# Gepeng18/Sentinel

Measured on AMD Instinct MI355X. Metric: admission decisions/sec at 1M rules Zipf(1.1), 1/2/4/8 GPU; % HBM peak, higher is better.
Workload: dtype int64

## Files before the change

### sentinel_amd/csrc/cluster.hip

```cpp
#include "cluster.hpp"
#include "cluster_exact.hpp"
#include "cparam_exact.hpp"

#include <cstdio>
#include <cstdlib>

#include <algorithm>
#include <type_traits>

namespace sga {

namespace {

constexpr int kThreads = 256;
constexpr int kItems = 16;
constexpr int kTileElems = kThreads * kItems;

enum : uint8_t { RUN_FAST = 0, RUN_DONE = 1 };

__device__ __forceinline__ uint64_t lanemask_lt64(int lane) { return (1ULL << lane) - 1ULL; }

__device__ __forceinline__ HashEntry slot_lookup(const ClusterState &st, int64_t fid) {
    uint32_t h = (uint32_t)hash_flow_id(fid) & st.hmask;
    for (uint32_t probe = 0; probe <= st.hmask; ++probe) {
// ... 1489 lines not shown
    const uint32_t hi = (uint32_t)__builtin_amdgcn_readlane((int)(uint32_t)((uint64_t)v >> 32), l);
    return (int64_t)(((uint64_t)hi << 32) | lo);
}

__device__ __forceinline__ uint32_t rank_hot(uint32_t *cw, uint32_t hid) {
    const uint32_t sh = (hid & 1u) << 4;
    return (atomicAdd(&cw[hid >> 1], 1u << sh) >> sh) & 0xFFFFu;
}


__device__ __forceinline__ uint32_t hot_count(const BatchScratch &sc) {
    return min(sc.hot_ctl[0], (uint32_t)kHot);
}

__device__ __forceinline__ uint32_t bucket_delta(uint32_t t, uint32_t W, uint32_t r0, double inv) {
    const uint64_t x = (uint64_t)r0 + t;
    int64_t q = (int64_t)((double)x * inv);
    const int64_t r = (int64_t)x - q * (int64_t)W;
    if (r < 0) --q;
    else if (r >= (int64_t)W) ++q;
    return (uint32_t)q;
}

__global__ __launch_bounds__(kThreads) void k_hot_precheck(ClusterState st, BatchScratch sc, const ReqIn in,
                                                           int64_t ts_base, uint32_t n, int pipelined) {
    if (blockIdx.x == 0 && st.dense_n) {
        const uint32_t W = st.wtab[threadIdx.x];
        WConst wc;
        wc.W = W;
        wc.r0 = (uint32_t)(ts_base % (int64_t)W);
        wc.inv = 1.0 / (double)W;
        sc.wconst[threadIdx.x] = wc;
    }
    const uint32_t h = blockIdx.x * kThreads + threadIdx.x;
    if (h < (uint32_t)kHot) {
        sc.plo[h] = 0;
        sc.phi[h] = 0;
    }
    if (h >= hot_count(sc) || n == 0) return;
    const int64_t W = (int64_t)sc.hot_ctl[2];
    const int64_t t0 = ts_base + (int64_t)in.ts_at(0);
    if (pipelined && h == 0 && t0 < (int64_t)*sc.tmax_all) atomicOr(&sc.counters[CTL_FLAGS], kFlagState);
    const int64_t ws0 = t0 - t0 % W;
    const uint32_t s = sc.hot_slot[h];
    const SlotParam P = st.param[s];
    bool bad = P.W != (int32_t)W || !P.active || P.S <= 1 || P.S > 64;
    const Rec R = rec_of(st, P);
    for (int j = 0; j < P.S && !bad; ++j) {
        const int64_t w = R.start(j);
        if (w != kAbsent && w > ws0) bad = true;
    }
    if (bad) atomicOr(&sc.counters[CTL_FLAGS], kFlagState);
}

constexpr uint32_t kKeyHot = 1u << 19;
constexpr uint32_t kPsGroups = 256;
constexpr int kKeyWaves = kHotSeg / kSubSeg;
constexpr int kKeyThreads = kKeyWaves * 64;
static_assert(kKeyWaves == kSubPerSeg, "one wave per compaction segment");
struct KeyShared {
    WConst wcs[256];
    uint16_t cnt[kKeyWaves][kHot];
    uint32_t s_np[kKeyWaves], s_bd[kKeyWaves], s_tm[kKeyWaves];
    uint32_t s_bmin, s_bmax;
    union {
        uint32_t hist0[2][256];
        uint32_t phist[kPartBins];
    };
};
template <int kPass, bool kDense, bool kNT = false, bool kPk = false>
__device__ __forceinline__ void hot_key(KeyShared &sh, const ClusterState &st, const BatchScratch &sc, const ReqIn in,
                                        int64_t ts_base, uint32_t n, uint64_t *__restrict__ out, int dbg,
                                        int d0, uint32_t *__restrict__ hist, uint32_t ntiles) {
    const int64_t *__restrict__ flow_id = in.flow;
    const int32_t *__restrict__ acquire = in.acq;
    const uint8_t *__restrict__ prio = in.prio;
    const uint32_t *__restrict__ ts_off = in.ts;
    const uint32_t *__restrict__ pk = in.pk;
    WConst *wcs = sh.wcs;
    const int pl = d0 < 0 ? -d0 : 0;
    if (pl) d0 = 0;
    const uint32_t dmask = (1u << d0) - 1u;
    auto &cnt = sh.cnt;
    uint32_t *s_np = sh.s_np, *s_bd = sh.s_bd;
    const uint32_t flags0 = sc.counters[CTL_FLAGS];
    if (kPass == 0 && (flags0 & kFlagState)) return;
    if (kPass == 1 && !(flags0 & (kFlagRerun | kFlagState))) return;
    const uint32_t nhot = kPass == 0 ? hot_count(sc) : 0u;
    const int lane = threadIdx.x & 63, wave = threadIdx.x >> 6;
    const uint64_t lt = lanemask_lt64(lane);
    if (kDense)
        for (int k = threadIdx.x; k < 256; k += kKeyThreads) wcs[k] = sc.wconst[k];
    for (int k = threadIdx.x; k < (pl ? kPartBins : 2 * 256); k += kKeyThreads) sh.phist[k] = 0;
    if (nhot) {
        uint4 *cz = reinterpret_cast<uint4 *>(&cnt[0][0]);
        for (int k = threadIdx.x; k < (int)(sizeof(cnt) / 16); k += kKeyThreads) cz[k] = make_uint4(0, 0, 0, 0);
    }
    if (threadIdx.x == 0) {
        sh.s_bmin = 0xFFFFFFFFu;
        sh.s_bmax = 0u;
    }
    __syncthreads();
    const uint32_t seg = blockIdx.x;
    const uint32_t sub = seg * kKeyWaves + wave;
    const uint32_t ubase = sub * kSubSeg;
    const bool active = ubase < n;
    uint16_t *c = cnt[wave];
    const uint32_t Wh = nhot ? sc.hot_ctl[2] : 1u;
    const uint32_t r0h = (uint32_t)(ts_base % (int64_t)Wh);
    const double invh = 1.0 / (double)Wh;
    const uint32_t Wc = (kDense && sc.hot_ctl[0]) ? sc.hot_ctl[2] : 1u;
    const uint32_t r0c = (uint32_t)(ts_base % (int64_t)Wc);
    const double invc = 1.0 / (double)Wc;
    uint32_t wflags = 0, nc = 0, np = 0, bdmax = 0, tmax_l = 0;
    const uint32_t send = min(n, ubase + (uint32_t)kSubSeg);
    uint32_t hc[kSubRounds];
#pragma unroll
    for (int r = 0; r < kSubRounds; ++r) hc[r] = kNoCode;
    if (active) {
        uint32_t ptso = ubase > 0 ? (kPk ? pk[3 * (size_t)(ubase - 1) + 1] : ts_off[ubase - 1]) : 0u;
        uint32_t pbd = (nhot && ubase > 0) ? min(bucket_delta(ptso, Wh, r0h, invh), (uint32_t)kHotBuckets - 1) : 0u;
        const bool use_prio = kPk || prio != nullptr;
        constexpr int nchunks = kSubRounds / kH1Chunk;
        struct Buf {
            int64_t f[kH1Chunk];
            int32_t a[kH1Chunk];
            uint32_t t[kH1Chunk], p[kH1Chunk], d[kH1Chunk], m[kH1Chunk];
            HashEntry e[kH1Chunk];
        };
        Buf B0, B1, B2;
        const uint8_t *pr_src = kPk ? nullptr : (use_prio ? prio : reinterpret_cast<const uint8_t *>(acquire));
        auto load = [&](int ch, Buf &B) {
#pragma unroll
            for (int u = 0; u < kH1Chunk; ++u) {
                const uint32_t i = min(ubase + (uint32_t)(ch * kH1Chunk + u) * 64 + lane, n - 1);
                if (kPk) {
                    const uint32_t *r = pk + 3 * (size_t)i;
                    uint32_t w0, w1, w2;
                    if (kNT) {
                        w0 = __builtin_nontemporal_load(r);
                        w1 = __builtin_nontemporal_load(r + 1);
                        w2 = __builtin_nontemporal_load(r + 2);
                    } else {
                        w0 = r[0];
                        w1 = r[1];
                        w2 = r[2];
// ... 127 lines not shown
                    ptso = lane_u32(B.t[u], 63);
                    if (valid && q >= (uint32_t)kHotBuckets) wflags |= kFlagBucket;
                    const uint32_t bdh = min(q, (uint32_t)kHotBuckets - 1);
                    if (valid) bdmax = max(bdmax, bdh);
                    if (i == 0) sc.counters[CTL_BDLO] = bdh;
                    const uint32_t pbk = wave_shr1(bdh, pbd);
                    if (valid && hp && bdh > pbk) {
                        for (uint32_t qq = pbk + 1; qq <= bdh; ++qq) sc.hbnd[qq] = i;
                        if (i & (uint32_t)(kHotSeg - 1)) {
                            atomicMin(&sh.s_bmin, pbk + 1);
                            atomicMax(&sh.s_bmax, bdh);
                        }
                    }
                    pbd = lane_u32(bdh, 63);
                    if (valid) hc[ch * kH1Chunk + u] = (kind == 2 ? (kKeyHot | hid | (p << 12)) : 0u) | (bdh << 13);
                }
                const bool emit = kind == 1;
                const uint64_t em = __ballot(emit);
                if (emit) {
                    if (kNT)
                        __builtin_nontemporal_store(el_pack(slot, bd6, p, a7, i),
                                                    &sc.el_tile[(size_t)ubase + nc + (uint32_t)__popcll(em & lt)]);
                    else
                        sc.el_tile[(size_t)ubase + nc + (uint32_t)__popcll(em & lt)] = el_pack(slot, bd6, p, a7, i);
                    if (d0) atomicAdd(&sh.hist0[wave >> 2][slot & dmask], 1u);
                    if (pl) atomicAdd(&sh.phist[slot >> pl], 1u);
                }
                nc += (uint32_t)__popcll(em);
            }
        };
        load(0, B0);
        lookup(B0);
        load(1, B1);
#pragma unroll
        for (int ch = 0; ch < nchunks; ch += 3) {
            lookup(B1);
            load(ch + 2, B2);
            process(B0, ch);
            if (ch + 1 >= nchunks) break;
            lookup(B2);
            load(ch + 3, B0);
            process(B1, ch + 1);
            if (ch + 2 >= nchunks) break;
            lookup(B0);
            load(ch + 4, B1);
            process(B2, ch + 2);
        }
        if (nhot && !(dbg & 4)) {
#pragma unroll
            for (int r = 0; r < kSubRounds; ++r) {
                const uint32_t i = ubase + (uint32_t)r * 64 + lane;
                const uint32_t kv = hc[r];
                const bool hot = i < send && (kv & kKeyHot);
                const uint32_t hid = kv & 0xFFFu, p = (kv >> 12) & 1u, bdh = (kv >> 13) & 63u;
                uint32_t r_in = 0;
                if (hot) r_in = rank_hot(reinterpret_cast<uint32_t *>(c), hid);
                np += (uint32_t)__popcll(__ballot(hot && p));
                hc[r] = hot ? ((p << 31) | hid | (r_in << 12) | (bdh << 25)) : kNoCode;
            }
        }
    }
    if (wflags) atomicOr(&sc.counters[CTL_FLAGS], wflags);
    if (nhot) {
bdmax = wave_max_u32(bdmax);
        if (lane == 0) {
            s_np[wave] = np;
            s_bd[wave] = bdmax;
        }
        __syncthreads();
        {
            uint32_t *cw = reinterpret_cast<uint32_t *>(&cnt[0][0]);
            uint32_t *row = reinterpret_cast<uint32_t *>(sc.hcnt + (size_t)seg * kHot);
            for (uint32_t k = threadIdx.x; k < (nhot + 1) / 2; k += kKeyThreads) {
                uint32_t run = 0;
#pragma unroll
                for (int w = 0; w < kKeyWaves; ++w) {
                    const uint32_t v = cw[w * (kHot / 2) + k];
                    cw[w * (kHot / 2) + k] = run;
                    run += v;
                }
                row[k] = run;
            }
        }
        if (threadIdx.x == 0) {
            uint32_t a = 0, m = 0;
            for (int w = 0; w < kKeyWaves; ++w) {
                a += s_np[w];
                m = max(m, s_bd[w]);
            }
            sc.seg_stat[kSegStat * seg] = a;
            sc.seg_stat[kSegStat * seg + 1] = m;
        }
        __syncthreads();
        if (active) {
            uint32_t npc = 0;
            for (int w = 0; w < wave; ++w) npc += s_np[w];
            const uint32_t pgper = (((n + kHotSeg - 1) / kHotSeg) + kPsGroups - 1) / kPsGroups;
#pragma unroll
            for (int r = 0; r < kSubRounds; ++r) {
                const uint32_t i = ubase + (uint32_t)r * 64 + lane;
                const uint32_t cd = hc[r];
                const bool hot = i < send && cd != kNoCode;
                const uint32_t hid = cd & 0xFFFu;
                const uint32_t r_seg = hot ? ((cd >> 12) & 0x1FFFu) + c[hid] : 0u;
                const bool pr = hot && (cd >> 31);
                if (i < send) sc.hcode[i] = hot ? ((cd & ~(0x1FFFu << 12)) | (r_seg << 12)) : kNoCode;
                const uint64_t em = __ballot(pr);
                if (pr) {
                    sc.pel_tile[(size_t)seg * kHotSeg + npc + (uint32_t)__popcll(em & lt)] = el_pack(hid, r_seg >> 7, 1u, r_seg & 127u, i);
                    atomicAdd(&sc.prow[(size_t)(seg / pgper) * kHot + hid], 1u);
                }
                npc += (uint32_t)__popcll(em);
            }
        }
        __syncthreads();
        const uint32_t b0 = sh.s_bmin, b1 = sh.s_bmax;
        uint32_t *pc = reinterpret_cast<uint32_t *>(&cnt[0][0]);
        for (uint32_t b = b0; b <= b1; ++b) {
            for (uint32_t k = threadIdx.x; k < nhot; k += kKeyThreads) pc[k] = 0;
            __syncthreads();
#pragma unroll
            for (int r = 0; r < kSubRounds; ++r) {
                const uint32_t cd = hc[r];
                if (ubase + (uint32_t)r * 64 + lane < send && cd != kNoCode && ((cd >> 25) & 63u) < b)
                    atomicAdd(&pc[cd & 0xFFFu], 1u);
            }
            __syncthreads();
            for (uint32_t k = threadIdx.x; k < nhot; k += kKeyThreads) sc.hpre[(size_t)b * kHot + k] = (uint16_t)pc[k];
            if (threadIdx.x == 0) atomicAdd(&sc.counters[CTL_NPRE], 1u);
            __syncthreads();
        }
    }
    {
tmax_l = wave_max_u32(tmax_l);
        if (lane == 0) sh.s_tm[wave] = tmax_l;
        __syncthreads();
        if (threadIdx.x == 0) {
            uint32_t m = 0;
            for (int w = 0; w < kKeyWaves; ++w) m = max(m, sh.s_tm[w]);
            sc.seg_stat[kSegStat * seg + 2] = m;
        }
    }
    if (lane == 0) sc.tile_nc[sub] = active ? nc : 0u;
    if (pl) {
        __syncthreads();
        for (uint32_t k = threadIdx.x; k < (uint32_t)kPartBins; k += kKeyThreads)
            hist[(size_t)seg * kPartBins + k] = sh.phist[k];
    }
    if (d0) {
        __syncthreads();
        for (uint32_t k = threadIdx.x; k < (2u << d0); k += kKeyThreads) {
            const uint32_t t = k >> d0, d = k & dmask, tile = seg * 2 + t;
            if (tile < ntiles) hist[(size_t)d * ntiles + tile] = sh.hist0[t][d];
        }
    }
}

__global__ __launch_bounds__(256) void k_part_colscan(BatchScratch sc, uint32_t nseg) {
    const uint32_t b = blockIdx.x * 256 + threadIdx.x;
    const uint32_t t0 = blockIdx.y * kPartGroup, t1 = min(nseg, t0 + kPartGroup);
    uint32_t acc = 0;
    for (uint32_t t = t0; t < t1; t += 8) {
        uint32_t v[8];
#pragma unroll
        for (int k = 0; k < 8; ++k) v[k] = t + k < t1 ? sc.phist[(size_t)(t + k) * kPartBins + b] : 0u;
#pragma unroll
        for (int k = 0; k < 8; ++k) {
            if (t + k < t1) sc.phist[(size_t)(t + k) * kPartBins + b] = acc;
            acc += v[k];
        }
    }
    sc.pgrp[(size_t)blockIdx.y * kPartBins + b] = acc;
}

__global__ __launch_bounds__(256) void k_part_binscan(BatchScratch sc, uint32_t ngroups) {
    __shared__ uint32_t ws[4];
    __shared__ uint32_t s_last;
    const int lane = threadIdx.x & 63, wave = threadIdx.x >> 6;
    const uint32_t b = blockIdx.x * 256 + threadIdx.x;
    uint32_t acc = 0;
    for (uint32_t g = 0; g < ngroups; g += 8) {
        uint32_t v[8];
#pragma unroll
        for (int k = 0; k < 8; ++k) v[k] = g + k < ngroups ? sc.pgrp[(size_t)(g + k) * kPartBins + b] : 0u;
#pragma unroll
        for (int k = 0; k < 8; ++k) {
            if (g + k < ngroups) sc.pgrp[(size_t)(g + k) * kPartBins + b] = acc;
            acc += v[k];
        }
    }
    sc.pstart[b] = acc;
    __threadfence();
    __syncthreads();
    if (threadIdx.x == 0) s_last = atomicAdd(&sc.pstart[kPartBins + 1], 1u) == gridDim.x - 1;
    __syncthreads();
    if (!s_last) return;
    __threadfence();
    constexpr int kPer = kPartBins / 256;
    uint32_t tot[kPer], ts = 0;
#pragma unroll
    for (int k = 0; k < kPer; ++k) {
        tot[k] = __hip_atomic_load(&sc.pstart[threadIdx.x * kPer + k], __ATOMIC_RELAXED, __HIP_MEMORY_SCOPE_AGENT);
        ts += tot[k];
    }
    uint32_t x = ts;
#pragma unroll
    for (int o = 1; o < 64; o <<= 1) {
        const uint32_t y = __shfl_up(x, o, 64);
        if (lane >= o) x += y;
    }
    if (lane == 63) ws[wave] = x;
    __syncthreads();
    uint32_t pre = x - ts;
    for (int w = 0; w < wave; ++w) pre += ws[w];
#pragma unroll
    for (int k = 0; k < kPer; ++k) {
        sc.pstart[threadIdx.x * kPer + k] = pre;
// ... 46 lines not shown
        for (int w = 0; w < kKeyWaves; ++w) {
            const uint32_t c = wc[w][b];
            wc[w][b] = (uint16_t)run;
            run += c;
        }
    }
    __syncthreads();
#pragma unroll
    for (int r = 0; r < kSubRounds; ++r) {
        if ((uint32_t)r * 64 >= nc) break;
        const bool valid = (uint32_t)r * 64 + lane < nc;
        const uint32_t b = el_slot(x[r]) >> lb;
        const uint64_t peers = match_lanes(b, kPartBits, valid);
        if (valid && !(dbg & 32)) out[gb[b] + wc[wave][b] + (uint32_t)__popcll(peers & lt)] = x[r];
        __builtin_amdgcn_wave_barrier();
        if (valid && (peers & lt) == 0) wc[wave][b] += (uint16_t)__popcll(peers);
        __builtin_amdgcn_wave_barrier();
    }
}

template <int kPass, bool kNT = false, bool kPk = false>
__global__ __launch_bounds__(kKeyThreads) __attribute__((amdgpu_waves_per_eu(4))) void k_hot_key_dense(
    ClusterState st, BatchScratch sc, ReqIn in, int64_t ts_base, uint32_t n, uint64_t *__restrict__ out, int dbg,
    int d0, uint32_t *__restrict__ hist, uint32_t ntiles) {
    __shared__ KeyShared sh;
    hot_key<kPass, true, kNT, kPk>(sh, st, sc, in, ts_base, n, out, dbg, d0, hist, ntiles);
}
template <int kPass, bool kPk = false>
__global__ __launch_bounds__(kKeyThreads) void k_hot_key_hash(
    ClusterState st, BatchScratch sc, ReqIn in, int64_t ts_base, uint32_t n, uint64_t *__restrict__ out, int dbg,
    int d0, uint32_t *__restrict__ hist, uint32_t ntiles) {
    __shared__ KeyShared sh;
    hot_key<kPass, false, false, kPk>(sh, st, sc, in, ts_base, n, out, dbg, d0, hist, ntiles);
}

__global__ __launch_bounds__(1024) void k_hot_mode(BatchScratch sc, uint32_t nsub, uint32_t nseg, int64_t ts_base) {
    __shared__ uint32_t red[4][16];
    const uint32_t f = sc.counters[CTL_FLAGS];
    const uint32_t nhot = (f & (kFlagRerun | kFlagState)) ? 0u : hot_count(sc);
    uint32_t ns = 0, np = 0, bd = 0, tm = 0;
    for (uint32_t k = threadIdx.x; k < nsub; k += 1024) ns += sc.tile_nc[k];
    for (uint32_t k = threadIdx.x; k < nseg; k += 1024) {
        if (nhot) {
            np += sc.seg_stat[kSegStat * k];
            bd = max(bd, sc.seg_stat[kSegStat * k + 1]);
        }
        tm = max(tm, sc.seg_stat[kSegStat * k + 2]);
    }
    ns = wave_sum_u32(ns);
    np = wave_sum_u32(np);
    bd = wave_max_u32(bd);
    tm = wave_max_u32(tm);
    if ((threadIdx.x & 63) == 0) {
        red[0][threadIdx.x >> 6] = ns;
        red[1][threadIdx.x >> 6] = np;
        red[2][threadIdx.x >> 6] = bd;
        red[3][threadIdx.x >> 6] = tm;
    }
    __syncthreads();
    if (threadIdx.x == 0) {
        uint32_t a = 0, b = 0, m = 0, t = 0;
        for (int w = 0; w < 16; ++w) {
            a += red[0][w];
            b += red[1][w];
            m = max(m, red[2][w]);
            t = max(t, red[3][w]);
        }
        atomicMax(sc.tmax_all, (unsigned long long)(ts_base + (int64_t)t));
        sc.counters[CTL_NSORT] = a;
        sc.counters[CTL_NPRIO] = b;
        sc.counters[CTL_NCOLD] = a;
        sc.counters[CTL_BDHI] = m;
        sc.counters[CTL_MODE] = nhot ? 1u : 0u;
    }
}

__global__ __launch_bounds__(kThreads) void k_hscan_group(BatchScratch sc, uint32_t nrows) {
    if (!sc.counters[CTL_MODE]) return;
    const uint32_t h = blockIdx.y * kThreads + threadIdx.x;
    if (h >= hot_count(sc)) return;
    const uint32_t r0 = blockIdx.x * kHotGroupRows;
    uint32_t s = 0;
#pragma unroll
    for (int k = 0; k < kHotGroupRows; ++k)
        if (r0 + k < nrows) s += sc.hcnt[(size_t)(r0 + k) * kHot + h];
    sc.hgsum[(size_t)blockIdx.x * kHot + h] = s;
}

__device__ __forceinline__ void psort_cols_one(const BatchScratch &sc, uint32_t h, uint32_t ngroups);
__global__ __launch_bounds__(kThreads) void k_hscan_mid(BatchScratch sc, uint32_t ngroups, uint32_t pgroups) {
    if (!sc.counters[CTL_MODE]) return;
    const uint32_t h = blockIdx.x * kThreads + threadIdx.x;
    if (pgroups) psort_cols_one(sc, h, pgroups);
    if (h >= hot_count(sc)) return;
    uint32_t acc = 0;
#pragma unroll 8
    for (uint32_t g = 0; g < ngroups; ++g) {
        const uint32_t v = sc.hgsum[(size_t)g * kHot + h];
        sc.hgsum[(size_t)g * kHot + h] = acc;
        acc += v;
    }
    sc.hot_tot[h] = acc;
}

__global__ __launch_bounds__(kThreads) void k_hscan_down(BatchScratch sc, uint32_t nrows) {
    if (!sc.counters[CTL_MODE]) return;
    const uint32_t h = blockIdx.y * kThreads + threadIdx.x;
// ... 1656 lines not shown
    const size_t nseg = hot_rows(cap) + 1;
    const size_t segs_alloc = ((nseg + kH1Waves - 1) / kH1Waves) * kH1Waves;
    size_t b = 0;
    b += 2 * align_up(cap * 8);
    b += 7 * align_up((cap + 1) * 4);
    b += align_up(cap + 1);
    b += align_up(cap * 4);
    b += align_up(cap * 8);
    b += align_up(cap * sizeof(RunOut));
    b += align_up(ntiles * kRunWaves * sizeof(RAgg));
    b += 2 * align_up(ntiles * sizeof(Agg)) + align_up(ntiles * 4);
    b += 2 * align_up(CTL_WORDS * 4);
    b += 2 * align_up(hist * 4) + align_up(scan_partials_needed(hist) * 4 + 64);
    b += align_up(scan_partials_needed(cap) * 4 + 64);
    b += align_up(kRadixGhistWords * 4) + align_up(64);
    b += align_up((size_t)nslots_cap * 2) + 2 * align_up(kHot * 4) + align_up(kHotCtlWords * 4);
    b += align_up(segs_alloc * kHotSeg * 8);
    b += align_up(segs_alloc * kSubPerSeg * 4);
    b += align_up(segs_alloc * kHotSeg * 8) + 2 * align_up((size_t)kPsGroups * kHot * 4);
    b += align_up(kHot * 4);
    b += 2 * align_up(cap * 8);
    b += 2 * align_up(hist * 4) + align_up(scan_partials_needed(hist) * 4 + 64);
    b += align_up(kRadixGhistWords * 4) + align_up(64);
    b += align_up(segs_alloc * kHotSeg * 4);
    b += align_up(segs_alloc * kHot * 2) + align_up(segs_alloc * kHot * 4);
    b += align_up(hot_groups(cap) * kHot * 4);
    b += align_up((size_t)kHotBuckets * kHot * 2) + align_up(kHotBuckets * 4);
    b += align_up((size_t)kHot * kHotBuckets * sizeof(HotRun));
    b += align_up((size_t)kHot * kHotBuckets * sizeof(uint4));
    b += align_up((size_t)kHot * kHotBuckets * sizeof(uint2));
    b += align_up(kHot * sizeof(double2));
    b += align_up(cap * 4);
    b += 3 * align_up(kHot * 4);
    b += align_up(256 * sizeof(WConst));
    b += align_up(segs_alloc * kSegStat * 4);
    b += align_up(64);
    b += align_up((size_t)kHotCand * 2 * 4);
    b += align_up(segs_alloc * kPartBins * 4);
    b += align_up(((segs_alloc + kPartGroup - 1) / kPartGroup) * kPartBins * 4);
    b += align_up((kPartBins + 2) * 4);
    return b;
}

void batch_scratch_carve(BatchScratch &sc, void *base, size_t cap, uint32_t nslots_cap) {
    const size_t ntiles = (cap + kTileElems - 1) / kTileElems + 1;
    const size_t hist = max_hist_entries(cap, nslots_cap);
    const size_t nseg = hot_rows(cap) + 1;
    const size_t segs_alloc = ((nseg + kH1Waves - 1) / kH1Waves) * kH1Waves;
    char *p = (char *)base;
    auto take = [&](size_t bytes) {
        void *r = p;
        p += align_up(bytes);
        return r;
    };
    sc.el[0] = (uint64_t *)take(cap * 8);
    sc.el[1] = (uint64_t *)take(cap * 8);
    sc.run_start = (uint32_t *)take((cap + 1) * 4);
    sc.run_slot = (uint32_t *)take((cap + 1) * 4);
    sc.run_idx0 = (uint32_t *)take((cap + 1) * 4);
    sc.run_cp = (uint32_t *)take((cap + 1) * 4);
    sc.run_p0 = (uint32_t *)take((cap + 1) * 4);
    sc.run_acq = (int32_t *)take((cap + 1) * 4);
    sc.flow_first_run = (uint32_t *)take((cap + 1) * 4);
    sc.run_bd = (uint8_t *)take(cap + 1);
    sc.plist = (uint32_t *)take(cap * 4);
    sc.deferred = (uint32_t *)take(cap * 8);
    sc.run_out = (RunOut *)take(cap * sizeof(RunOut));
// ... 9 lines not shown
    sc.radix.partial = (uint32_t *)take(scan_partials_needed(hist) * 4 + 64);
    sc.lim_partial = (uint32_t *)take(scan_partials_needed(cap) * 4 + 64);
    sc.radix.ghist = (uint32_t *)take(kRadixGhistWords * 4);
    sc.radix.err = (uint32_t *)take(64);
    sc.hot_of = (uint16_t *)take((size_t)nslots_cap * 2);
    sc.hot_slot = (uint32_t *)take(kHot * 4);
    sc.hot_next = (uint32_t *)take(kHot * 4);
    sc.hot_ctl = (uint32_t *)take(kHotCtlWords * 4);
    sc.el_tile = (uint64_t *)take(segs_alloc * kHotSeg * 8);
    sc.tile_nc = (uint32_t *)take(segs_alloc * kSubPerSeg * 4);
    sc.pel_tile = (uint64_t *)take(segs_alloc * kHotSeg * 8);
    sc.prow = (uint32_t *)take((size_t)kPsGroups * kHot * 4);
    sc.ppre = (uint32_t *)take((size_t)kPsGroups * kHot * 4);
    sc.ptot = (uint32_t *)take(kHot * 4);
    SGA_HIP_CHECK(hipMemset(sc.prow, 0, (size_t)kPsGroups * kHot * 4));
    sc.pel[0] = (uint64_t *)take(cap * 8);
    sc.pel[1] = (uint64_t *)take(cap * 8);
    (void)take(hist * 4); (void)take(hist * 4); (void)take(scan_partials_needed(hist) * 4 + 64);
    (void)take(kRadixGhistWords * 4); (void)take(64);
    sc.hcode = (uint32_t *)take(segs_alloc * kHotSeg * 4);
    sc.hcnt = (uint16_t *)take(segs_alloc * kHot * 2);
    sc.hbase = (uint32_t *)take(segs_alloc * kHot * 4);
    sc.hgsum = (uint32_t *)take(hot_groups(cap) * kHot * 4);
    sc.hpre = (uint16_t *)take((size_t)kHotBuckets * kHot * 2);
    sc.hbnd = (uint32_t *)take(kHotBuckets * 4);
    sc.hrun = (HotRun *)take((size_t)kHot * kHotBuckets * sizeof(HotRun));
    sc.hfin = (uint4 *)take((size_t)kHot * kHotBuckets * sizeof(uint4));
    sc.hfs = (uint2 *)take((size_t)kHot * kHotBuckets * sizeof(uint2));
    sc.hthr = (double2 *)take(kHot * sizeof(double2));
    sc.prank = (uint32_t *)take(cap * 4);
    sc.plo = (uint32_t *)take(kHot * 4);
    sc.phi = (uint32_t *)take(kHot * 4);
    sc.hot_tot = (uint32_t *)take(kHot * 4);
    sc.wconst = (WConst *)take(256 * sizeof(WConst));
    sc.seg_stat = (uint32_t *)take(segs_alloc * kSegStat * 4);
    sc.tmax_all = (unsigned long long *)take(64);
    sc.hot_cand = (uint32_t *)take((size_t)kHotCand * 2 * 4);
    sc.phist = (uint32_t *)take(segs_alloc * kPartBins * 4);
    sc.pgrp = (uint32_t *)take(((segs_alloc + kPartGroup - 1) / kPartGroup) * kPartBins * 4);
    sc.pstart = (uint32_t *)take((kPartBins + 2) * 4);
    sc.cap = cap;
}

__device__ __forceinline__ uint32_t probe_mix(uint32_t x) {
    x ^= x >> 16;
    x *= 0x7feb352dU;
    x ^= x >> 15;
    x *= 0x846ca68bU;
    x ^= x >> 16;
    return x;
}
__global__ __launch_bounds__(kThreads) void k_lds_order_probe(uint32_t *bad) {
    __shared__ uint32_t cw[kThreads / 64][kHot / 2];
    const int lane = threadIdx.x & 63, w = threadIdx.x >> 6;
    const uint32_t K = 1u << (blockIdx.x % 13);
    const int mode = (blockIdx.x / 13) % 3;
    for (int k = lane; k < kHot / 2; k += 64) cw[w][k] = 0;
    __builtin_amdgcn_wave_barrier();
    const uint64_t lt = lanemask_lt64(lane);
    uint32_t nb = 0;
    for (uint32_t r = 0; r < 32; ++r) {
        const uint32_t x = probe_mix((blockIdx.x * 1315423911u) ^ (r * 2654435761u) ^ (threadIdx.x * 97u));
        uint32_t hid = x % K;
        if (mode == 1 && (x & 1u)) hid = 7 % K;
        const bool act = mode == 2 ? ((x >> 8) & 1u) : true;
        const uint32_t sh = (hid & 1u) << 4;
        const uint32_t before = (cw[w][hid >> 1] >> sh) & 0xFFFFu;
// ... 82 lines not shown
static void prio_sort(BatchScratch &sc, uint32_t nseg, hipStream_t s, bool cols_done = false) {
    const uint32_t ngroups = ps_groups_h(nseg);
    if (fz_debug() & 512) hipLaunchKernelGGL(k_psort_dbgcount, dim3(kPsGroups), dim3(64), 0, s, sc, nseg);
    if (!cols_done) hipLaunchKernelGGL(k_psort_cols, dim3(kHot / 256), dim3(256), 0, s, sc, ngroups);
    hipLaunchKernelGGL(k_psort_scatter, dim3(kPsGroups), dim3(64), 0, s, sc, nseg, sc.pel[0], fz_debug());
    if (fz_debug() & 512) hipLaunchKernelGGL(k_psort_verify, dim3(4), dim3(256), 0, s, sc, sc.pel[0]);
    sc.pel_sorted = sc.pel[0];
}

static void classify_hot(const ClusterState &st, BatchScratch &sc, const ReqIn &in, int64_t ts_base, uint32_t n,
                         uint64_t *out, hipStream_t s, bool clean, bool pipelined) {
    const int bits = hot_key_bits(st);
    const uint32_t nseg = (n + kHotSeg - 1) / kHotSeg;
    const uint32_t ngroups = (nseg + kHotGroupRows - 1) / kHotGroupRows;
    if (!clean) SGA_HIP_CHECK(hipMemsetAsync(sc.counters, 0, CTL_WORDS * 4, s));
    hipLaunchKernelGGL(k_hot_precheck, dim3(kHot / kThreads), dim3(kThreads), 0, s, st, sc, in, ts_base, n,
                       pipelined ? 1 : 0);
    static const bool key_nt = !(getenv("SGA_KEY_NT") && atoi(getenv("SGA_KEY_NT")) == 0);
    const bool pk = in.pk != nullptr;
    auto hka = st.dense_n ? (pk ? (key_nt ? k_hot_key_dense<0, true, true> : k_hot_key_dense<0, false, true>)
                                : (key_nt ? k_hot_key_dense<0, true, false> : k_hot_key_dense<0, false, false>))
                          : (pk ? k_hot_key_hash<0, true> : k_hot_key_hash<0, false>);
    auto hkb = st.dense_n ? (pk ? k_hot_key_dense<1, false, true> : k_hot_key_dense<1, false, false>)
                          : (pk ? k_hot_key_hash<1, true> : k_hot_key_hash<1, false>);
    const int dsort = radix64_digit_bits(bits);
    sc.part_lb = cold_part_lb(bits);
    const int d0 = sc.part_lb ? -sc.part_lb : (dsort <= 8 ? dsort : 0);
    const uint32_t ntiles_sort = (uint32_t)radix64_tiles(n);
    uint32_t *khist = sc.part_lb ? sc.phist : sc.radix.hist;
    hipLaunchKernelGGL(hka, dim3(nseg), dim3(kKeyThreads), 0, s, st, sc, in, ts_base, n, out, fz_debug(), d0, khist,
                       ntiles_sort);
    hipLaunchKernelGGL(hkb, dim3(nseg), dim3(kKeyThreads), 0, s, st, sc, in, ts_base, n, out, fz_debug(), d0, khist,
                       ntiles_sort);
    hipLaunchKernelGGL(k_hot_mode, dim3(1), dim3(1024), 0, s, sc, nseg * kKeyWaves, nseg, ts_base);
    const bool ovl = hot_overlap() && !(fz_debug() & 16);
    sc.sched2 = ovl && !pipelined && hot_sched() == 2;
    if (sc.sched2) {
        side_stream_init(sc);
        SGA_HIP_CHECK(hipEventRecord(sc.ev_fork0, s));
        SGA_HIP_CHECK(hipStreamWaitEvent(sc.side, sc.ev_fork0, 0));
        if (sc.part_lb) {
            const uint32_t pg = (nseg + kPartGroup - 1) / kPartGroup;
            hipLaunchKernelGGL(k_part_colscan, dim3(kPartBins / 256, pg), dim3(256), 0, sc.side, sc, nseg);
            hipLaunchKernelGGL(k_part_binscan, dim3(kPartBins / 256), dim3(256), 0, sc.side, sc, pg);
            hipLaunchKernelGGL(k_part_scatter, dim3(8 * ((nseg + 7) / 8)), dim3(kKeyThreads), 0, sc.side, sc, nseg,
                               sc.part_lb, sc.el[0], fz_debug());
            sc.el_sorted = sc.el[0];
        } else {
            const int np = radix_sort_u64_tiled(sc.el_tile, sc.tile_nc, sc.counters + CTL_NSORT, sc.el[0], sc.el[1], n,
                                                kSlotShift, bits, sc.radix, sc.side, d0 > 0);
            sc.el_sorted = (np & 1) ? sc.el[0] : sc.el[1];
        }
        SGA_HIP_CHECK(hipEventRecord(sc.ev_fork, sc.side));
        prio_sort(sc, nseg, s);
        hipLaunchKernelGGL(k_hscan_group, dim3(ngroups, kHot / kThreads), dim3(kThreads), 0, s, sc, nseg);
        hipLaunchKernelGGL(k_hscan_mid, dim3(kHot / kThreads), dim3(kThreads), 0, s, sc, ngroups, 0u);
        hipLaunchKernelGGL(k_hscan_down, dim3(ngroups, kHot / kThreads), dim3(kThreads), 0, s, sc, nseg);
        const uint32_t pgrid = std::max<uint32_t>(1, std::min<uint32_t>((n + kThreads - 1) / kThreads, 1024));
        hipLaunchKernelGGL(k_prio_rank, dim3(pgrid), dim3(kThreads), 0, s, st, sc, sc.pel_sorted);
        hipLaunchKernelGGL(k_hot_flows, dim3(kHot / kH1Waves), dim3(kThreads), 0, s, st, sc, ts_base);
        SGA_HIP_CHECK(hipEventRecord(sc.ev_mid, s));
        SGA_HIP_CHECK(hipStreamWaitEvent(sc.side2, sc.ev_mid, 0));
        launch_hot_final(st, sc, n, sc.pel_sorted, out, sc.side2);
        SGA_HIP_CHECK(hipEventRecord(sc.ev_join, sc.side2));
        sc.hot_early = true;
        return;
    }
    const bool scans_first = ovl && !pipelined && hot_sched() == 3;
    static const bool hot_one = !getenv("SGA_HOT_ONE") || atoi(getenv("SGA_HOT_ONE")) == 1;
    hipStream_t hs = s;
    if (ovl && !pipelined && !scans_first && hot_one) {
        side_stream_init(sc);
        SGA_HIP_CHECK(hipEventRecord(sc.ev_fork0, s));
        SGA_HIP_CHECK(hipStreamWaitEvent(sc.side, sc.ev_fork0, 0));
        hipStream_t hs1 = hs = sc.side;
        hipLaunchKernelGGL(k_hscan_group, dim3(ngroups, kHot / kThreads), dim3(kThreads), 0, hs1, sc, nseg);
        hipLaunchKernelGGL(k_hscan_mid, dim3(kHot / kThreads), dim3(kThreads), 0, hs1, sc, ngroups, ps_groups_h(nseg));
// ... 6 lines not shown
        side_stream_init(sc);
        SGA_HIP_CHECK(hipEventRecord(sc.ev_fork0, s));
        if (!scans_first) {
            SGA_HIP_CHECK(hipStreamWaitEvent(sc.side, sc.ev_fork0, 0));
            hs = sc.side;
        }
    }
    hipStream_t ps = hs;
    if (ovl) {
        SGA_HIP_CHECK(hipStreamWaitEvent(sc.side2, sc.ev_fork0, 0));
        ps = sc.side2;
    }
    static const bool prio_late = !getenv("SGA_PRIO_LATE") || atoi(getenv("SGA_PRIO_LATE")) == 1;
    auto prio_sort = [&] { sga::prio_sort(sc, nseg, ps); };
    if (!prio_late) prio_sort();
    hipLaunchKernelGGL(k_hscan_group, dim3(ngroups, kHot / kThreads), dim3(kThreads), 0, hs, sc, nseg);
    hipLaunchKernelGGL(k_hscan_mid, dim3(kHot / kThreads), dim3(kThreads), 0, hs, sc, ngroups, 0u);
    hipLaunchKernelGGL(k_hscan_down, dim3(ngroups, kHot / kThreads), dim3(kThreads), 0, hs, sc, nseg);
    if (prio_late) prio_sort();
    if (scans_first) {
        SGA_HIP_CHECK(hipEventRecord(sc.ev_fork, s));
        SGA_HIP_CHECK(hipStreamWaitEvent(sc.side, sc.ev_fork, 0));
        hs = sc.side;
    }
    if (ovl) {
        SGA_HIP_CHECK(hipEventRecord(sc.ev_prio, ps));
        SGA_HIP_CHECK(hipStreamWaitEvent(hs, sc.ev_prio, 0));
    }
    sc.hot_early = ovl && !pipelined;
    if (sc.hot_early) hot_side(st, sc, ts_base, n, out, hs, true);
    }
    if (sc.part_lb) {
        const uint32_t ngroups = (nseg + kPartGroup - 1) / kPartGroup;
        hipLaunchKernelGGL(k_part_colscan, dim3(kPartBins / 256, ngroups), dim3(256), 0, s, sc, nseg);
        hipLaunchKernelGGL(k_part_binscan, dim3(kPartBins / 256), dim3(256), 0, s, sc, ngroups);
        hipLaunchKernelGGL(k_part_scatter, dim3(8 * ((nseg + 7) / 8)), dim3(kKeyThreads), 0, s, sc, nseg, sc.part_lb,
                           sc.el[0], fz_debug());
        sc.el_sorted = sc.el[0];
    } else {
        const int np = radix_sort_u64_tiled(sc.el_tile, sc.tile_nc, sc.counters + CTL_NSORT, sc.el[0], sc.el[1], n,
                                            kSlotShift, bits, sc.radix, s, d0 > 0);
        sc.el_sorted = (np & 1) ? sc.el[0] : sc.el[1];
    }
    if (ovl && !sc.hot_early) {
        SGA_HIP_CHECK(hipEventRecord(sc.ev_fork, hs));
        SGA_HIP_CHECK(hipStreamWaitEvent(s, sc.ev_fork, 0));
    }
}

static void decide_hot(const ClusterState &st, BatchScratch &sc, const ReqIn &in, int64_t ts_base, uint32_t n,
                       uint64_t *out, hipStream_t s) {
    const uint32_t invalid_key = st.nslots;
    const uint64_t *el = sc.el_sorted, *pel = sc.pel_sorted;
    const bool ovl = hot_overlap() && !(fz_debug() & 16);
    if (sc.sched2) SGA_HIP_CHECK(hipStreamWaitEvent(s, sc.ev_fork, 0));
    if (!sc.hot_early) {
        hipStream_t hs = s;
        if (ovl) {
            side_stream_init(sc);
            SGA_HIP_CHECK(hipEventRecord(sc.ev_fork0, s));
            SGA_HIP_CHECK(hipStreamWaitEvent(sc.side, sc.ev_fork0, 0));
            hs = sc.side;
        }
        hot_side(st, sc, ts_base, n, out, hs, ovl);
    }
    cold_stage(st, sc, el, n, sc.counters + CTL_NCOLD, invalid_key, in, ts_base, 0, std::max<uint32_t>(sc.hot_min, 1),
               out, s);
    if (fz_debug() & 16) {
        unsigned long long ph[8];
        SGA_HIP_CHECK(hipMemcpyFromSymbolAsync(ph, HIP_SYMBOL(g_fz_phase), sizeof(ph), 0, hipMemcpyDeviceToHost, s));
        SGA_HIP_CHECK(hipStreamSynchronize(s));
        const unsigned long long z[8] = {0, 0, 0, 0, 0, 0, 0, 0};
        SGA_HIP_CHECK(hipMemcpyToSymbolAsync(HIP_SYMBOL(g_fz_phase), z, sizeof(z), 0, hipMemcpyHostToDevice, s));
        if (ph[7])
            fprintf(stderr, "fz phases (wall_clock64 ticks per workgroup, %llu wgs): order %.0f runs %.0f flows %.0f results %.0f\n",
                    ph[7], (double)ph[3] / ph[7], (double)ph[0] / ph[7], (double)ph[1] / ph[7], (double)ph[2] / ph[7]);
    }
    if (!ovl) {
        launch_hot_final(st, sc, n, pel, out, s);
    } else if (!tail_early()) {
        SGA_HIP_CHECK(hipStreamWaitEvent(s, sc.ev_join, 0));
    } else {
        SGA_HIP_CHECK(hipStreamWaitEvent(s, sc.ev_mid, 0));
    }
    const uint32_t sb = 64;
    static const int next = getenv("SGA_HOT_NEXT") ? atoi(getenv("SGA_HOT_NEXT")) : 3;
    if (next == 3) {
        hipLaunchKernelGGL(k_hot_next_a, dim3(sb), dim3(kThreads), 0, s, st, sc, std::max<uint32_t>(sc.hot_min, 1));
        hipLaunchKernelGGL(k_hot_pick, dim3(sb), dim3(kThreads), 0, s, st, sc, sc.hot_min);
        if (ovl && tail_early()) SGA_HIP_CHECK(hipStreamWaitEvent(s, sc.ev_join, 0));
        hipLaunchKernelGGL(k_hot_fin, dim3(1), dim3(kFinThreads), 0, s, st, sc);
    } else if (next == 4) {
        hipLaunchKernelGGL(k_hot_hist, dim3(sb), dim3(kThreads), 0, s, st, sc, std::max<uint32_t>(sc.hot_min, 1));
        hipLaunchKernelGGL(k_hot_clear, dim3(kHot / kThreads), dim3(kThreads), 0, s, st, sc);
        hipLaunchKernelGGL(k_hot_pick, dim3(sb), dim3(kThreads), 0, s, st, sc, sc.hot_min);
        if (ovl && tail_early()) SGA_HIP_CHECK(hipStreamWaitEvent(s, sc.ev_join, 0));
        hipLaunchKernelGGL(k_hot_fin, dim3(1), dim3(kFinThreads), 0, s, st, sc);
    } else {
        hipLaunchKernelGGL(k_hot_next_a, dim3(sb), dim3(kThreads), 0, s, st, sc, std::max<uint32_t>(sc.hot_min, 1));
        if (ovl && tail_early()) SGA_HIP_CHECK(hipStreamWaitEvent(s, sc.ev_join, 0));
// ... 348 lines not shown
```

### sentinel_amd/csrc/cluster.hpp

```cpp
#pragma once
#include "../../include/sentinel_amd.h"
#include "common.hpp"
#include "radix_sort.hpp"

namespace sga {

struct SlotParam {
    double thr;
    double thr_simple;
    double isec;
    uint32_t boff;
    int32_t S;
    int32_t W;
    int32_t interval;
    int32_t active;
    int32_t ns;
};

struct SlotOcc {
    int64_t occ_pass;
    int64_t occ_preq;
    int32_t has_occ;
    int32_t pad;
};
// ... 68 lines not shown
};

struct HotRun {
    int64_t s0;
    double thr;
    double isec;
    uint32_t f;
    uint32_t start;
    uint32_t n;
    uint32_t p0;
    uint32_t cpf;
    uint32_t cw;
    uint16_t wait;
    uint8_t ok;
    uint8_t pad;
    uint32_t pad2[3];
};
static_assert(sizeof(HotRun) == 64, "hot run record");

constexpr int kHot = 4096;
constexpr uint16_t kColdId = 0xFFFF;
constexpr uint32_t kNoSlot = 0xFFFFFFFFu;
constexpr int kHotCtlWords = 128;
constexpr int kHotSeg = 8192;
constexpr int kSubSeg = 1024;
constexpr int kHotBuckets = 64;
constexpr int kHotGroupRows = 16;
constexpr int kHotCand = 1 << 16;
constexpr int kSegStat = 4;
constexpr int kPartBits = 11;
constexpr int kPartBins = 1 << kPartBits;
constexpr int kPartGroup = 64;
constexpr int kPartMaxLow = 10;

enum : int {
    CTL_NVALID = 0, CTL_NRUNS = 1, CTL_NFLOWS = 2, CTL_LIMITED = 4, CTL_LIMRUNS = 5, CTL_DEFERRED = 6,
    CTL_FLAGS = 16,
    CTL_NPRIO = 19,
    CTL_NSORT = 20,
    CTL_NCOLD = 21,
    CTL_NPRE = 22,
    CTL_BDLO = 23,
    CTL_BDHI = 24,
    CTL_MODE = 25,
    CTL_HOTERR = 26,
    CTL_WORDS = 64
};
enum : uint32_t {
    kFlagUnsorted = 1,
    kFlagMixed = 2,
    kFlagBucket = 4,
    kFlagHotKey = 8,
    kFlagRerun = 15,
    kFlagState = 16
};

struct WConst {
    uint32_t W, r0;
    double inv;
};

struct BatchScratch {
    uint64_t *el[2];
    uint32_t *run_start, *run_slot, *run_idx0, *run_cp, *run_p0;
    int32_t *run_acq;
    uint8_t *run_bd;
    uint32_t *flow_first_run;
    uint32_t *plist;
    uint32_t *deferred;
    RunOut *run_out;
    RAgg *wave_carry;
    void *tile_agg;
    void *tile_carry;
    uint32_t *tile_valid;
    uint32_t *counters;
    uint32_t *counters_last;
    int counters_clean = 0;
    uint32_t *lim_partial;
// ... 158 lines not shown
```

Before: 21.33 billion.

## Fold hot-mode reduction and partition scans into last-block-done epilogues

Removes the separate single-block k_hot_mode launch by having the last hot_key block, found through an atomic done counter, perform the segment-stat reduction. It merges k_part_colscan and k_part_binscan into one kernel with the same last-block pattern, and precomputes the hot window constants once in k_hot_precheck. Cross-block visibility relies on agent-scope relaxed stores and loads plus vmcnt waits. The aim is fewer kernel launches and serial gaps on the critical path. In exchange it adds atomics, needs done counters that are reset correctly between batches, and adds debug phase timers.

```diff
diff --git a/sentinel_amd/csrc/cluster.hip b/sentinel_amd/csrc/cluster.hip
--- a/sentinel_amd/csrc/cluster.hip
+++ b/sentinel_amd/csrc/cluster.hip
@@ -1545,6 +1545,13 @@
         wc.inv = 1.0 / (double)W;
         sc.wconst[threadIdx.x] = wc;
     }
+    if (blockIdx.x == 0 && threadIdx.x == 0) {
+        WConst wc;
+        wc.W = sc.hot_ctl[0] ? sc.hot_ctl[2] : 1u;
+        wc.r0 = (uint32_t)(ts_base % (int64_t)wc.W);
+        wc.inv = 1.0 / (double)wc.W;
+        sc.wconst[kWcHot] = wc;
+    }
     const uint32_t h = blockIdx.x * kThreads + threadIdx.x;
     if (h < (uint32_t)kHot) {
         sc.plo[h] = 0;
@@ -1574,13 +1581,75 @@
 struct KeyShared {
     WConst wcs[256];
     uint16_t cnt[kKeyWaves][kHot];
-    uint32_t s_np[kKeyWaves], s_bd[kKeyWaves], s_tm[kKeyWaves];
+    uint32_t s_np[kKeyWaves], s_bd[kKeyWaves], s_tm[kKeyWaves], s_nc[kKeyWaves];
     uint32_t s_bmin, s_bmax;
+    uint32_t s_last;
+    uint32_t red[4][kKeyWaves];
     union {
         uint32_t hist0[2][256];
         uint32_t phist[kPartBins];
     };
 };
+__device__ unsigned long long g_key_phase[8];
+__device__ __forceinline__ void key_mark(int dbg, int ph, unsigned long long &t) {
+    if (!(dbg & 1024)) return;
+    const unsigned long long now = wall_clock64();
+    if (threadIdx.x == 0) {
+        atomicAdd(&g_key_phase[ph], now - t);
+        if (ph == 5) atomicAdd(&g_key_phase[7], 1ull);
+    }
+    t = now;
+}
+
+__device__ __forceinline__ void st_agent(uint32_t *p, uint32_t v) {
+    __hip_atomic_store(p, v, __ATOMIC_RELAXED, __HIP_MEMORY_SCOPE_AGENT);
+}
+__device__ __forceinline__ uint32_t ld_agent(const uint32_t *p) {
+    return __hip_atomic_load(p, __ATOMIC_RELAXED, __HIP_MEMORY_SCOPE_AGENT);
+}
+
+__device__ __forceinline__ void key_mode(KeyShared &sh, const BatchScratch &sc, uint32_t nseg, int64_t ts_base) {
+    const uint32_t f = ld_agent(&sc.counters[CTL_FLAGS]);
+    const uint32_t nhot = (f & (kFlagRerun | kFlagState)) ? 0u : hot_count(sc);
+    uint32_t ns = 0, np = 0, bd = 0, tm = 0;
+#pragma unroll 4
+    for (uint32_t k = threadIdx.x; k < nseg; k += kKeyThreads) {
+        const uint32_t a = ld_agent(&sc.seg_stat[kSegStat * k]), m = ld_agent(&sc.seg_stat[kSegStat * k + 1]);
+        tm = max(tm, ld_agent(&sc.seg_stat[kSegStat * k + 2]));
+        ns += ld_agent(&sc.seg_stat[kSegStat * k + 3]);
+        if (nhot) {
+            np += a;
+            bd = max(bd, m);
+        }
+    }
+    ns = wave_sum_u32(ns);
+    np = wave_sum_u32(np);
+    bd = wave_max_u32(bd);
+    tm = wave_max_u32(tm);
+    if ((threadIdx.x & 63) == 0) {
+        sh.red[0][threadIdx.x >> 6] = ns;
+        sh.red[1][threadIdx.x >> 6] = np;
+        sh.red[2][threadIdx.x >> 6] = bd;
+        sh.red[3][threadIdx.x >> 6] = tm;
+    }
+    __syncthreads();
+    if (threadIdx.x == 0) {
+        uint32_t a = 0, b = 0, m = 0, t = 0;
+        for (int w = 0; w < kKeyWaves; ++w) {
+            a += sh.red[0][w];
+            b += sh.red[1][w];
+            m = max(m, sh.red[2][w]);
+            t = max(t, sh.red[3][w]);
+        }
+        atomicMax(sc.tmax_all, (unsigned long long)(ts_base + (int64_t)t));
+        sc.counters[CTL_NSORT] = a;
+        sc.counters[CTL_NPRIO] = b;
+        sc.counters[CTL_NCOLD] = a;
+        sc.counters[CTL_BDHI] = m;
+        sc.counters[CTL_MODE] = nhot ? 1u : 0u;
+    }
+}
+
 template <int kPass, bool kDense, bool kNT = false, bool kPk = false>
 __device__ __forceinline__ void hot_key(KeyShared &sh, const ClusterState &st, const BatchScratch &sc, const ReqIn in,
                                         int64_t ts_base, uint32_t n, uint64_t *__restrict__ out, int dbg,
@@ -1602,8 +1671,17 @@
     const uint32_t nhot = kPass == 0 ? hot_count(sc) : 0u;
     const int lane = threadIdx.x & 63, wave = threadIdx.x >> 6;
     const uint64_t lt = lanemask_lt64(lane);
+    unsigned long long tk = (dbg & 1024) ? wall_clock64() : 0ull;
     if (kDense)
         for (int k = threadIdx.x; k < 256; k += kKeyThreads) wcs[k] = sc.wconst[k];
+    const WConst wch = sc.wconst[kWcHot];
+    const uint32_t Wh = __builtin_amdgcn_readfirstlane(wch.W), r0h = __builtin_amdgcn_readfirstlane(wch.r0);
+    const uint32_t Wc = Wh, r0c = r0h;
+    const uint64_t invb = __double_as_longlong(wch.inv);
+    const double invh = __longlong_as_double(
+        ((uint64_t)(uint32_t)__builtin_amdgcn_readfirstlane((int)(uint32_t)(invb >> 32)) << 32) |
+        (uint32_t)__builtin_amdgcn_readfirstlane((int)(uint32_t)invb));
+    const double invc = invh;
     for (int k = threadIdx.x; k < (pl ? kPartBins : 2 * 256); k += kKeyThreads) sh.phist[k] = 0;
     if (nhot) {
         uint4 *cz = reinterpret_cast<uint4 *>(&cnt[0][0]);
@@ -1614,17 +1692,12 @@
         sh.s_bmax = 0u;
     }
     __syncthreads();
+    key_mark(dbg, 0, tk);
     const uint32_t seg = blockIdx.x;
     const uint32_t sub = seg * kKeyWaves + wave;
     const uint32_t ubase = sub * kSubSeg;
     const bool active = ubase < n;
     uint16_t *c = cnt[wave];
-    const uint32_t Wh = nhot ? sc.hot_ctl[2] : 1u;
-    const uint32_t r0h = (uint32_t)(ts_base % (int64_t)Wh);
-    const double invh = 1.0 / (double)Wh;
-    const uint32_t Wc = (kDense && sc.hot_ctl[0]) ? sc.hot_ctl[2] : 1u;
-    const uint32_t r0c = (uint32_t)(ts_base % (int64_t)Wc);
-    const double invc = 1.0 / (double)Wc;
     uint32_t wflags = 0, nc = 0, np = 0, bdmax = 0, tmax_l = 0;
     const uint32_t send = min(n, ubase + (uint32_t)kSubSeg);
     uint32_t hc[kSubRounds];
@@ -1818,6 +1891,10 @@
         load(0, B0);
         lookup(B0);
         load(1, B1);
+        if (dbg & 1024) {
+            __builtin_amdgcn_s_waitcnt(0x0F70);
+            key_mark(dbg, 1, tk);
+        }
 #pragma unroll
         for (int ch = 0; ch < nchunks; ch += 3) {
             lookup(B1);
@@ -1832,6 +1909,7 @@
             load(ch + 4, B1);
             process(B2, ch + 2);
         }
+        key_mark(dbg, 2, tk);
         if (nhot && !(dbg & 4)) {
 #pragma unroll
             for (int r = 0; r < kSubRounds; ++r) {
@@ -1847,6 +1925,7 @@
         }
     }
     if (wflags) atomicOr(&sc.counters[CTL_FLAGS], wflags);
+    key_mark(dbg, 3, tk);
     if (nhot) {
 bdmax = wave_max_u32(bdmax);
         if (lane == 0) {
@@ -1874,8 +1953,8 @@
                 a += s_np[w];
                 m = max(m, s_bd[w]);
             }
-            sc.seg_stat[kSegStat * seg] = a;
-            sc.seg_stat[kSegStat * seg + 1] = m;
+            st_agent(&sc.seg_stat[kSegStat * seg], a);
+            st_agent(&sc.seg_stat[kSegStat * seg + 1], m);
         }
         __syncthreads();
         if (active) {
@@ -1917,14 +1996,22 @@
             __syncthreads();
         }
     }
+    key_mark(dbg, 4, tk);
     {
 tmax_l = wave_max_u32(tmax_l);
-        if (lane == 0) sh.s_tm[wave] = tmax_l;
+        if (lane == 0) {
+            sh.s_tm[wave] = tmax_l;
+            sh.s_nc[wave] = active ? nc : 0u;
+        }
         __syncthreads();
         if (threadIdx.x == 0) {
-            uint32_t m = 0;
-            for (int w = 0; w < kKeyWaves; ++w) m = max(m, sh.s_tm[w]);
-            sc.seg_stat[kSegStat * seg + 2] = m;
+            uint32_t m = 0, a = 0;
+            for (int w = 0; w < kKeyWaves; ++w) {
+                m = max(m, sh.s_tm[w]);
+                a += sh.s_nc[w];
+            }
+            st_agent(&sc.seg_stat[kSegStat * seg + 2], m);
+            st_agent(&sc.seg_stat[kSegStat * seg + 3], a);
         }
     }
     if (lane == 0) sc.tile_nc[sub] = active ? nc : 0u;
@@ -1940,10 +2027,22 @@
             if (tile < ntiles) hist[(size_t)d * ntiles + tile] = sh.hist0[t][d];
         }
     }
-}
-
-__global__ __launch_bounds__(256) void k_part_colscan(BatchScratch sc, uint32_t nseg) {
+    key_mark(dbg, 5, tk);
+    asm volatile("s_waitcnt vmcnt(0)" ::: "memory");
+    __syncthreads();
+    if (threadIdx.x == 0) sh.s_last = atomicAdd(&sc.counters[CTL_KEYDONE + kPass], 1u) == gridDim.x - 1;
+    __syncthreads();
+    if (!sh.s_last) return;
+    key_mode(sh, sc, gridDim.x, ts_base);
+    if ((dbg & 1024) && threadIdx.x == 0) atomicAdd(&g_key_phase[6], wall_clock64() - tk);
+}
+
+__global__ __launch_bounds__(256) void k_part_scan(BatchScratch sc, uint32_t nseg) {
+    __shared__ uint32_t ws[4];
+    __shared__ uint32_t s_last;
+    const int lane = threadIdx.x & 63, wave = threadIdx.x >> 6;
     const uint32_t b = blockIdx.x * 256 + threadIdx.x;
+    const uint32_t ngroups = gridDim.y;
     const uint32_t t0 = blockIdx.y * kPartGroup, t1 = min(nseg, t0 + kPartGroup);
     uint32_t acc = 0;
     for (uint32_t t = t0; t < t1; t += 8) {
@@ -1956,19 +2055,18 @@
             acc += v[k];
         }
     }
-    sc.pgrp[(size_t)blockIdx.y * kPartBins + b] = acc;
-}
-
-__global__ __launch_bounds__(256) void k_part_binscan(BatchScratch sc, uint32_t ngroups) {
-    __shared__ uint32_t ws[4];
-    __shared__ uint32_t s_last;
-    const int lane = threadIdx.x & 63, wave = threadIdx.x >> 6;
-    const uint32_t b = blockIdx.x * 256 + threadIdx.x;
-    uint32_t acc = 0;
+    st_agent(&sc.pgrp[(size_t)blockIdx.y * kPartBins + b], acc);
+    asm volatile("s_waitcnt vmcnt(0)" ::: "memory");
+    __syncthreads();
+    if (threadIdx.x == 0) s_last = atomicAdd(&sc.counters[CTL_PARTDONE + blockIdx.x], 1u) == ngroups - 1;
+    __syncthreads();
+    if (!s_last) return;
+    acc = 0;
     for (uint32_t g = 0; g < ngroups; g += 8) {
         uint32_t v[8];
 #pragma unroll
-        for (int k = 0; k < 8; ++k) v[k] = g + k < ngroups ? sc.pgrp[(size_t)(g + k) * kPartBins + b] : 0u;
+        for (int k = 0; k < 8; ++k)
+            v[k] = g + k < ngroups ? ld_agent(&sc.pgrp[(size_t)(g + k) * kPartBins + b]) : 0u;
 #pragma unroll
         for (int k = 0; k < 8; ++k) {
             if (g + k < ngroups) sc.pgrp[(size_t)(g + k) * kPartBins + b] = acc;
@@ -2081,47 +2179,6 @@
     int d0, uint32_t *__restrict__ hist, uint32_t ntiles) {
     __shared__ KeyShared sh;
     hot_key<kPass, false, false, kPk>(sh, st, sc, in, ts_base, n, out, dbg, d0, hist, ntiles);
-}
-
-__global__ __launch_bounds__(1024) void k_hot_mode(BatchScratch sc, uint32_t nsub, uint32_t nseg, int64_t ts_base) {
-    __shared__ uint32_t red[4][16];
-    const uint32_t f = sc.counters[CTL_FLAGS];
-    const uint32_t nhot = (f & (kFlagRerun | kFlagState)) ? 0u : hot_count(sc);
-    uint32_t ns = 0, np = 0, bd = 0, tm = 0;
-    for (uint32_t k = threadIdx.x; k < nsub; k += 1024) ns += sc.tile_nc[k];
-    for (uint32_t k = threadIdx.x; k < nseg; k += 1024) {
-        if (nhot) {
-            np += sc.seg_stat[kSegStat * k];
-            bd = max(bd, sc.seg_stat[kSegStat * k + 1]);
-        }
-        tm = max(tm, sc.seg_stat[kSegStat * k + 2]);
-    }
-    ns = wave_sum_u32(ns);
-    np = wave_sum_u32(np);
-    bd = wave_max_u32(bd);
-    tm = wave_max_u32(tm);
-    if ((threadIdx.x & 63) == 0) {
-        red[0][threadIdx.x >> 6] = ns;
-        red[1][threadIdx.x >> 6] = np;
-        red[2][threadIdx.x >> 6] = bd;
-        red[3][threadIdx.x >> 6] = tm;
-    }
-    __syncthreads();
-    if (threadIdx.x == 0) {
-        uint32_t a = 0, b = 0, m = 0, t = 0;
-        for (int w = 0; w < 16; ++w) {
-            a += red[0][w];
-            b += red[1][w];
-            m = max(m, red[2][w]);
-            t = max(t, red[3][w]);
-        }
-        atomicMax(sc.tmax_all, (unsigned long long)(ts_base + (int64_t)t));
-        sc.counters[CTL_NSORT] = a;
-        sc.counters[CTL_NPRIO] = b;
-        sc.counters[CTL_NCOLD] = a;
-        sc.counters[CTL_BDHI] = m;
-        sc.counters[CTL_MODE] = nhot ? 1u : 0u;
-    }
 }
 
 __global__ __launch_bounds__(kThreads) void k_hscan_group(BatchScratch sc, uint32_t nrows) {
@@ -3844,7 +3901,7 @@
     b += align_up(kHot * sizeof(double2));
     b += align_up(cap * 4);
     b += 3 * align_up(kHot * 4);
-    b += align_up(256 * sizeof(WConst));
+    b += align_up((kWcHot + 1) * sizeof(WConst));
     b += align_up(segs_alloc * kSegStat * 4);
     b += align_up(64);
     b += align_up((size_t)kHotCand * 2 * 4);
@@ -3920,7 +3977,7 @@
     sc.plo = (uint32_t *)take(kHot * 4);
     sc.phi = (uint32_t *)take(kHot * 4);
     sc.hot_tot = (uint32_t *)take(kHot * 4);
-    sc.wconst = (WConst *)take(256 * sizeof(WConst));
+    sc.wconst = (WConst *)take((kWcHot + 1) * sizeof(WConst));
     sc.seg_stat = (uint32_t *)take(segs_alloc * kSegStat * 4);
     sc.tmax_all = (unsigned long long *)take(64);
     sc.hot_cand = (uint32_t *)take((size_t)kHotCand * 2 * 4);
@@ -4069,7 +4126,6 @@
                        ntiles_sort);
     hipLaunchKernelGGL(hkb, dim3(nseg), dim3(kKeyThreads), 0, s, st, sc, in, ts_base, n, out, fz_debug(), d0, khist,
                        ntiles_sort);
-    hipLaunchKernelGGL(k_hot_mode, dim3(1), dim3(1024), 0, s, sc, nseg * kKeyWaves, nseg, ts_base);
     const bool ovl = hot_overlap() && !(fz_debug() & 16);
     sc.sched2 = ovl && !pipelined && hot_sched() == 2;
     if (sc.sched2) {
@@ -4078,8 +4134,7 @@
         SGA_HIP_CHECK(hipStreamWaitEvent(sc.side, sc.ev_fork0, 0));
         if (sc.part_lb) {
             const uint32_t pg = (nseg + kPartGroup - 1) / kPartGroup;
-            hipLaunchKernelGGL(k_part_colscan, dim3(kPartBins / 256, pg), dim3(256), 0, sc.side, sc, nseg);
-            hipLaunchKernelGGL(k_part_binscan, dim3(kPartBins / 256), dim3(256), 0, sc.side, sc, pg);
+            hipLaunchKernelGGL(k_part_scan, dim3(kPartBins / 256, pg), dim3(256), 0, sc.side, sc, nseg);
             hipLaunchKernelGGL(k_part_scatter, dim3(8 * ((nseg + 7) / 8)), dim3(kKeyThreads), 0, sc.side, sc, nseg,
                                sc.part_lb, sc.el[0], fz_debug());
             sc.el_sorted = sc.el[0];
@@ -4152,8 +4207,7 @@
     }
     if (sc.part_lb) {
         const uint32_t ngroups = (nseg + kPartGroup - 1) / kPartGroup;
-        hipLaunchKernelGGL(k_part_colscan, dim3(kPartBins / 256, ngroups), dim3(256), 0, s, sc, nseg);
-        hipLaunchKernelGGL(k_part_binscan, dim3(kPartBins / 256), dim3(256), 0, s, sc, ngroups);
+        hipLaunchKernelGGL(k_part_scan, dim3(kPartBins / 256, ngroups), dim3(256), 0, s, sc, nseg);
         hipLaunchKernelGGL(k_part_scatter, dim3(8 * ((nseg + 7) / 8)), dim3(kKeyThreads), 0, s, sc, nseg, sc.part_lb,
                            sc.el[0], fz_debug());
         sc.el_sorted = sc.el[0];
@@ -4186,6 +4240,18 @@
     }
     cold_stage(st, sc, el, n, sc.counters + CTL_NCOLD, invalid_key, in, ts_base, 0, std::max<uint32_t>(sc.hot_min, 1),
                out, s);
+    if (fz_debug() & 1024) {
+        unsigned long long ph[8];
+        SGA_HIP_CHECK(hipMemcpyFromSymbolAsync(ph, HIP_SYMBOL(g_key_phase), sizeof(ph), 0, hipMemcpyDeviceToHost, s));
+        SGA_HIP_CHECK(hipStreamSynchronize(s));
+        const unsigned long long z[8] = {0, 0, 0, 0, 0, 0, 0, 0};
+        SGA_HIP_CHECK(hipMemcpyToSymbolAsync(HIP_SYMBOL(g_key_phase), z, sizeof(z), 0, hipMemcpyHostToDevice, s));
+        if (ph[7])
+            fprintf(stderr, "key phases (wall_clock64 ticks per segment, %llu segments): setup %.1f first %.1f stream %.1f "
+                            "rank %.1f fixup %.1f rows %.1f; mode %llu\n",
+                    ph[7], (double)ph[0] / ph[7], (double)ph[1] / ph[7], (double)ph[2] / ph[7], (double)ph[3] / ph[7],
+                    (double)ph[4] / ph[7], (double)ph[5] / ph[7], ph[6]);
+    }
     if (fz_debug() & 16) {
         unsigned long long ph[8];
         SGA_HIP_CHECK(hipMemcpyFromSymbolAsync(ph, HIP_SYMBOL(g_fz_phase), sizeof(ph), 0, hipMemcpyDeviceToHost, s));
diff --git a/sentinel_amd/csrc/cluster.hpp b/sentinel_amd/csrc/cluster.hpp
--- a/sentinel_amd/csrc/cluster.hpp
+++ b/sentinel_amd/csrc/cluster.hpp
@@ -124,6 +124,7 @@
 constexpr int kPartBins = 1 << kPartBits;
 constexpr int kPartGroup = 64;
 constexpr int kPartMaxLow = 10;
+constexpr int kWcHot = 256;
 
 enum : int {
     CTL_NVALID = 0, CTL_NRUNS = 1, CTL_NFLOWS = 2, CTL_LIMITED = 4, CTL_LIMRUNS = 5, CTL_DEFERRED = 6,
@@ -136,6 +137,8 @@
     CTL_BDHI = 24,
     CTL_MODE = 25,
     CTL_HOTERR = 26,
+    CTL_KEYDONE = 27,
+    CTL_PARTDONE = 32,
     CTL_WORDS = 64
 };
 enum : uint32_t {
```

Measured after the change: 21.39 billion, median of 6. No clear change (+0.3%).
